# CaptainCuong/Efficient-GNN

Measured on NVIDIA B200. Metric: chebyshev_wavelet_nnz_k_f_per_s, higher is better.
Workload: dtype f32

## Files before the change

### efficient-gnn_b200/_cabi.py

```python
from __future__ import annotations

import ctypes as C
import os
import threading

_HERE = os.path.dirname(os.path.abspath(__file__))
LIB_PATH = os.environ.get("EGNN_LIB_PATH") or os.path.join(_HERE, "lib", "libegnn_b200.so")
ABI_VERSION = 9

_P, _I32, _I64, _F32, _SZ = C.c_void_p, C.c_int32, C.c_int64, C.c_float, C.c_size_t
SYMBOLS = {
    "egnn_abi_version": (C.c_int, []),
    "egnn_last_error": (C.c_char_p, []),
    "egnn_device_info": (C.c_int, [_P, _P, _P]),
    "egnn_dense_to_csr_count": (C.c_int, [_P, _I64, _I64, _P, _P, _P]),
    "egnn_dense_to_csr_fill": (C.c_int, [_P, _I64, _I64, _P, _P, _P, _P]),
    "egnn_graph_prep": (C.c_int, [_P, _P, _P, _I64, _P, _P, _P, _P, _P, _P, _P, _P, _P]),
    "egnn_degree_rows": (C.c_int, [_P, _P, _P, _I64, _I64, _I64, _P, _P, _P, _P, _P]),
    "egnn_graph_prep_finish": (C.c_int, [_P, _P, _P, _I64, _P, _P, _P, _P, _P]),
    "egnn_calibration_metrics_ws_bytes": (_SZ, [_I32, _I32]),
    "egnn_calibration_metrics": (C.c_int, [_P, _I32, _P, _P, _I64, _I32, _I32, _P, _P, _SZ, _P]),
    "egnn_temperature_head": (C.c_int, [_P, _P, _P, _P, _P, _P, _P, _P, _I64, _I32, _I32, _I32, _P]),
    "egnn_gcn_propagate": (C.c_int, [_P, _P, _P, _P, _P, _P, _P, _I64, _I32, _P, _P, _P, _I32, _P]),
    "egnn_gcn_target_logits": (C.c_int, [_P, _P, _P, _P, _P, _P, _I32, _I64, _I32, _I32, _P, _P, _P, _P, _P, _I32, _P]),
# ... 45 lines not shown
                                          _I32, _I32, _P, _P, _P, _I32, _P]),
    "egnn_cheb_adjoint_sharded": (C.c_int, [_P, _P, _P, _P, _P, _P, _P, _P, _P, _P, _P, _P, _P,
                                            _I64, _I64, _I64, _I64, _I32, _I32, _I32, _I32, _P, _F32, _F32, _I32,
                                            _P, _P, _P, _I32, _P]),
    "egnn_wide_adjoint_sharded": (C.c_int, [_P, _P, _P, _P, _P, _P, _P, _P, _I64, _I64, _I64, _I32, _I32, _I32, _I32,
                                            _P, _F32, _F32, _P, _P, _P, _I32, _P, _P]),
}


class SellPlanStruct(C.Structure):
    _fields_ = [("n", C.c_int32), ("n_blocks", C.c_int32), ("col_block", C.c_int32), ("lmax", C.c_int32),
                ("n_cols", C.c_int32), ("row0", C.c_int32), ("n_cta", C.c_int32), ("reserved", C.c_int32),
                ("n_slices", C.c_int64), ("n_vrows", C.c_int64), ("n_entries", C.c_int64), ("n_rowv", C.c_int64),
                ("slice_off", C.c_void_p), ("blk_slice_ptr", C.c_void_p), ("idx", C.c_void_p),
                ("rv_ptr", C.c_void_p), ("vslot", C.c_void_p), ("cta_info", C.c_void_p), ("vpart", C.c_void_p),
                ("sched", C.c_void_p), ("stamps", C.c_void_p)]


MAX_RANKS = 16
IPC_HANDLE_BYTES = 64


class PeerWindowStruct(C.Structure):
    _fields_ = [("rank", C.c_int32), ("world", C.c_int32), ("rows_per", C.c_int64), ("f", C.c_int32),
                ("reserved", C.c_int32), ("base", C.c_void_p * MAX_RANKS)]


class EgnnError(RuntimeError):
    """A non-zero status from libegnn_b200 (message from egnn_last_error)."""


# ... 72 lines not shown
```

### efficient-gnn_b200/csrc/egnn_cabi.cu

```cuda
#include <stdarg.h>
#include <stdlib.h>

#include "adjoint.cuh"
#include "cheb.cuh"
#include "common.cuh"
#include "head.cuh"
#include "metrics.cuh"
#include "peer.cuh"
#include "prep.cuh"
#include "sell.cuh"
#include "sell_step.cuh"
#include "structure_grad.cuh"
#include "surrogate.cuh"
#include "blocked.cuh"
#include "wide.cuh"

namespace egnn {

static thread_local char g_err[512] = {0};
char* last_error_buf() { return g_err; }
void set_error(const char* fmt, ...) {
    va_list ap;
    va_start(ap, fmt);
    vsnprintf(g_err, sizeof(g_err), fmt, ap);
// ... 220 lines not shown
static void fill_peer_push(PeerPush& pp, const egnn_peer_window* w, int which, bool has_data, bool wait_first) {
    pp.world = w->world; pp.rank = w->rank; pp.wait_first = wait_first; pp.has_data = has_data;
    char* own = (char*)w->base[w->rank];
    for (int r = 0; r < w->world; ++r) {
        pp.dst[r] = peer_operand(w, r, which);
        pp.flag[r] = (unsigned*)((char*)w->base[r] + kPeerFlagsOff) + w->rank;
    }
    pp.local_flags = (unsigned*)(own + kPeerFlagsOff);
    pp.epoch = (unsigned*)(own + kPeerEpochOff);
    pp.done_ctr = (unsigned*)(own + kPeerDoneOff);
    pp.error = (unsigned*)(own + kPeerErrorOff);
}

static void step_fill_plan(SellStepParams& sp, const egnn_sell_plan* pl) {
    sp.idx = pl->idx; sp.slice_off = pl->slice_off; sp.blk_slice_ptr = pl->blk_slice_ptr; sp.vslot = pl->vslot;
    sp.cta_info = pl->cta_info; sp.rv_ptr = pl->rv_ptr; sp.vpart = pl->vpart; sp.sched = pl->sched;
    sp.stamps = (unsigned long long*)pl->stamps;
    sp.trace = pl->reserved;
    sp.n_cta = pl->n_cta; sp.C = pl->n_blocks; sp.CB = pl->col_block; sp.n_cols = pl->n_cols;
    sp.n_rows = pl->n; sp.row0 = pl->row0;
}

static void step_fill_peer(SellStepParams& sp, const egnn_peer_window* w) {
    sp.world = w->world; sp.rank = w->rank; sp.rows_per = w->rows_per;
    char* own = (char*)w->base[w->rank];
    for (int r = 0; r < w->world; ++r) sp.flag_at[r] = (unsigned*)((char*)w->base[r] + kPeerFlagsOff) + w->rank;
    sp.local_flags = (unsigned*)(own + kPeerFlagsOff);
    sp.epoch = (unsigned*)(own + kPeerEpochOff);
    sp.error = (unsigned*)(own + kPeerErrorOff);
}

// ... 35 lines not shown
    return EGNN_OK;
}

static int device_sm_count() {
    int dev = 0, sms = kSmCountB200;
    if (cudaGetDevice(&dev) == cudaSuccess) cudaDeviceGetAttribute(&sms, cudaDevAttrMultiProcessorCount, dev);
    return sms;
}

}

using namespace egnn;

extern "C" {

int egnn_abi_version(void) { return 9; }

const char* egnn_last_error(void) { return last_error_buf(); }

int egnn_device_info(int32_t* sm_count, int32_t* cc_major, int32_t* cc_minor) {
    int dev = 0;
    int rc = check_cuda(cudaGetDevice(&dev), "cudaGetDevice");
    if (rc) return rc;
    cudaDeviceProp prop;
    rc = check_cuda(cudaGetDeviceProperties(&prop, dev), "cudaGetDeviceProperties");
    if (rc) return rc;
    if (sm_count) *sm_count = prop.multiProcessorCount;
    if (cc_major) *cc_major = prop.major;
    if (cc_minor) *cc_minor = prop.minor;
    if (prop.major != 10) {
        set_error("libegnn_b200 is built for sm_100a only; device is sm_%d%d", prop.major, prop.minor);
// ... 248 lines not shown
    float* tbuf[2] = {(float*)ws, (float*)(ws + slab)};
    float* ybuf[2] = {(float*)(ws + 2 * slab), (float*)(ws + 3 * slab)};

    if (t_all_or_null) {
        rc = check_cuda(cudaMemcpyAsync(t_all_or_null, x0, sizeof(float) * slab_elems, cudaMemcpyDeviceToDevice, st), "copy T0");
        if (rc) return rc;
    }
    if (cfg.prescaled && !sell_plan) {
        prescale_kernel<<<grid_for((int64_t)slab_elems, 256), 256, 0, st>>>(x0, dinv, ybuf[0], n, f, 0);
        EGNN_LAUNCH_CHECK("prescale_kernel launch");
    }

    if (sell_plan) {
        EGNN_REQUIRE(f == 1 && vals_or_null == nullptr, "the SELL plan serves F = 1 on a binary adjacency");
        EGNN_REQUIRE(sell_plan->n == n && sell_plan->n_cols == n && sell_plan->row0 == 0 && sell_plan->vpart && sell_plan->slice_off && sell_plan->blk_slice_ptr &&
                     sell_plan->rv_ptr && sell_plan->vslot && sell_plan->cta_info && sell_plan->sched, "SELL plan does not match the graph or is not filled");
        SellStepParams sp{};
        step_fill_plan(sp, sell_plan);
        sp.delta = p.delta;
        sp.w_base = w_base_or_null; sp.rowsum_base = rowsum_base_or_null; sp.patch_x0 = default_signal ? 1 : 0;
        sp.dinv = dinv; sp.iso = iso; sp.x0 = x0;
        sp.operand_first = y0_or_null;
        sp.operand[0] = ybuf[0]; sp.operand[1] = ybuf[1];
        sp.ydst[0][0] = ybuf[0]; sp.ydst[1][0] = ybuf[1]; sp.n_dst = 1;
        sp.tbuf[0] = tbuf[0]; sp.tbuf[1] = tbuf[1]; sp.t_all = t_all_or_null; sp.out = out;
        sp.normalize = normalize_l1; sp.a = op_scale; sp.b = op_shift;
        sp.world = 1; sp.rank = 0; sp.rows_per = n;
        if (order_events_host) {
            rc = check_cuda(cudaEventRecord((cudaEvent_t)order_events_host[0], st), "event record");
            if (rc) return rc;
        }
// ... 615 lines not shown
    rc = check_cuda(cub::DeviceScan::ExclusiveSum(w.cub_temp, tb, w.nvrow, w.rv_ptr, (int)(n + 1), st), "scan nvrow"); if (rc) return rc;
    sell_emit_kernel<<<(unsigned)ceil_div64(cn, 256), 256, 0, st>>>((int)n, C, lmax, w.seg_start, w.seg_cnt, w.nv, w.u_off,
                                                                   w.rv_ptr, w.key, w.uval, w.vsrc, w.vslot, w.vrow);
    EGNN_LAUNCH_CHECK("sell_emit_kernel launch");
    tb = w.cub_bytes;
    rc = check_cuda(cub::DeviceRadixSort::SortPairs(w.cub_temp, tb, w.key, w.key_sorted, w.uval, w.perm, (int)w.umax, 0, 32, st), "sort vrows");
    if (rc) return rc;
    sell_blocks_kernel<<<1, 32, 0, st>>>((int)n, C, w.u_off, w.q_ptr, w.vp_ptr, w.bsp, w.bstride, w.totals);
    EGNN_LAUNCH_CHECK("sell_blocks_kernel launch");
    sell_slice_kernel<<<(unsigned)ceil_div64(w.smax, 256), 256, 0, st>>>(C, lmax, w.key_sorted, w.q_ptr, w.bsp, w.bstride, w.totals, w.slice_sz);
    EGNN_LAUNCH_CHECK("sell_slice_kernel launch");
    tb = w.cub_bytes;
    rc = check_cuda(cub::DeviceScan::ExclusiveSum(w.cub_temp, tb, w.slice_sz, w.slice_off, (int)(w.smax + 1), st), "scan slices"); if (rc) return rc;
    sell_totals_kernel<<<1, 32, 0, st>>>(w.slice_off, w.rv_ptr, (int)n, w.totals);
    EGNN_LAUNCH_CHECK("sell_totals_kernel launch");
    int64_t tot[8];
    rc = check_cuda(cudaMemcpyAsync(tot, w.totals, 64, cudaMemcpyDeviceToHost, st), "copy totals"); if (rc) return rc;
    rc = check_cuda(cudaStreamSynchronize(st), "sync"); if (rc) return rc;
    plan->n = (int32_t)n;
    plan->n_cta = device_sm_count();
    plan->n_vrows = tot[kTotV];
    plan->n_slices = tot[kTotSlices];
    plan->n_entries = tot[kTotEntries];
    plan->n_rowv = tot[kTotRowV];
    return EGNN_OK;
}

int egnn_sell_fill(const int32_t* rowptr, const int32_t* colidx, int64_t n, int64_t nnz,
                   const egnn_sell_plan* plan, void* workspace, size_t workspace_bytes, egnn_stream_t stream) {
    int rc = sell_check_geometry(n, nnz, plan);
    if (rc) return rc;
    (void)rowptr;
    EGNN_REQUIRE(plan->slice_off && plan->blk_slice_ptr && plan->rv_ptr && plan->cta_info && plan->sched, "plan buffers not allocated");
    EGNN_REQUIRE(plan->n_cta >= 1 && plan->n_cta <= 4096, "n_cta out of range");
    EGNN_REQUIRE(plan->n_entries == 0 || plan->idx, "plan idx not allocated");
    EGNN_REQUIRE(plan->n_vrows == 0 || plan->vslot, "plan vslot not allocated");
    const int C = plan->n_blocks, CB = plan->col_block, lmax = plan->lmax;
    SellWs w = sell_ws_layout(workspace, n, nnz, C, lmax);
    if (!workspace || workspace_bytes < w.total_bytes) {
        set_error("sell workspace too small: need %zu bytes, got %zu", w.total_bytes, workspace_bytes);
        return EGNN_ERR_WORKSPACE;
    }
    cudaStream_t st = (cudaStream_t)stream;
    rc = check_cuda(cudaMemcpyAsync(plan->slice_off, w.slice_off, 4 * (plan->n_slices + 1), cudaMemcpyDeviceToDevice, st), "copy slice_off"); if (rc) return rc;
    rc = check_cuda(cudaMemcpyAsync(plan->blk_slice_ptr, w.bsp, 4 * (C + 1), cudaMemcpyDeviceToDevice, st), "copy blk_slice_ptr"); if (rc) return rc;
    rc = check_cuda(cudaMemcpyAsync(plan->rv_ptr, w.rv_ptr, 4 * (n + 1), cudaMemcpyDeviceToDevice, st), "copy rv_ptr"); if (rc) return rc;
    sell_cta_blocks_kernel<<<1, 32, 0, st>>>(w.slice_off, w.bsp, C, plan->n_cta, plan->cta_info, plan->sched);
    EGNN_LAUNCH_CHECK("sell_cta_blocks_kernel launch");
    sell_row_cost_kernel<<<(unsigned)ceil_div64(n + 1, 256), 256, 0, st>>>(w.rv_ptr, (int)n, w.nvrow);
    EGNN_LAUNCH_CHECK("sell_row_cost_kernel launch");
    size_t tb = w.cub_bytes;
    rc = check_cuda(cub::DeviceScan::ExclusiveSum(w.cub_temp, tb, w.nvrow, w.nv, (int)(n + 1), st), "scan row costs"); if (rc) return rc;
    sell_cta_rows_kernel<<<(unsigned)ceil_div64(plan->n_cta + 1, 128), 128, 0, st>>>(w.nv, (int)n, plan->n_cta,
                                                                                 plan->cta_info + 2 * plan->n_cta + kSellMaxBlocks);
    EGNN_LAUNCH_CHECK("sell_cta_rows_kernel launch");
    if (plan->n_slices > 0) {
        rc = check_cuda(cudaFuncSetAttribute(sell_fill_kernel, cudaFuncAttributeMaxDynamicSharedMemorySize, (int)kSellFillSmem),
                        "cudaFuncSetAttribute(sell_fill_kernel)");
        if (rc) return rc;
        sell_fill_kernel<<<(unsigned)ceil_div64(plan->n_slices, kSellFillWarps), kSellFillWarps * 32, kSellFillSmem, st>>>(
            colidx, C, CB, lmax, (int)plan->n_slices, w.key_sorted, w.perm, w.vsrc, w.vslot, w.vrow, w.q_ptr, w.vp_ptr,
            w.bsp, w.bstride, w.slice_off, plan->idx, plan->vslot, plan->row0);
        EGNN_LAUNCH_CHECK("sell_fill_kernel launch");
    }
    return EGNN_OK;
}

int egnn_sell_step_sharded(const egnn_sell_plan* plan, const float* dinv_full, const uint8_t* iso_full,
                           const float* x0_local, const float* y_first_full, float* y_slab0, float* y_slab1,
                           float* tbuf0, float* tbuf1, float* t_all_or_null, float* out_local,
                           int32_t order_begin, int32_t order_end, int32_t k_max, int32_t n_scales,
                           const float* coeffs_host, float op_scale, float op_shift, int32_t normalize_l1,
                           const int32_t* delta_row_host, const int32_t* delta_col_host,
                           const float* delta_val_host, int32_t n_delta,
                           const float* w_base_or_null, const float* rowsum_base_or_null, int32_t default_signal,
                           const egnn_peer_window* win, egnn_stream_t stream) {
    EGNN_REQUIRE(plan && dinv_full && iso_full && out_local && coeffs_host, "null pointer");
    EGNN_REQUIRE((w_base_or_null == nullptr) == (rowsum_base_or_null == nullptr), "w_base and rowsum_base come together");
    EGNN_REQUIRE(plan->vpart && plan->slice_off && plan->blk_slice_ptr && plan->rv_ptr && plan->vslot && plan->cta_info && plan->sched,
                 "SELL plan is not filled");
    EGNN_REQUIRE(order_begin >= 1 && order_begin <= order_end && order_end <= k_max && k_max <= EGNN_MAX_ORDER, "bad order range");
    EGNN_REQUIRE(n_scales >= 1 && n_scales <= EGNN_MAX_SCALES, "n_scales out of range");
    EGNN_REQUIRE(plan->n == 0 || x0_local, "T_0 rows missing");
    EGNN_REQUIRE(t_all_or_null || k_max == 1 || (tbuf0 && tbuf1), "T buffers missing");
    const bool fused = win && win->world > 1;
    if (win) {
        int rc = peer_check(win);
        if (rc) return rc;
        EGNN_REQUIRE(win->f == 1 && (int64_t)win->world * win->rows_per >= plan->n_cols &&
                     (int64_t)plan->row0 + plan->n <= (int64_t)win->world * win->rows_per, "window does not fit the plan");
    } else {
        EGNN_REQUIRE(plan->n == plan->n_cols || (order_begin == order_end && y_first_full),
                     "a row shard without an exchange window runs one order per call on a gathered operand");
        EGNN_REQUIRE(order_end == k_max || (y_slab0 && y_slab1), "operand slabs missing");
// ... 516 lines not shown
```

### efficient-gnn_b200/csrc/sell.cuh

```cuda
#pragma once

#include <cub/device/device_radix_sort.cuh>
#include <cub/device/device_scan.cuh>

#include "cheb.cuh"
#include "common.cuh"
#include "peer.cuh"

namespace egnn {

constexpr int kSellThreads = 1024;
constexpr int kSellThreadsPerCta = kSellThreads;
constexpr int kSellCtrStride = 32;
constexpr int kSellSchedWords = 64 * kSellCtrStride + 64;
constexpr int kSellSliceRows = 32;
constexpr int kSellGroup = 8;
constexpr int kSellMaxBlocks = 64;

enum SellTotals { kTotU = 0, kTotV = 1, kTotSlices = 2, kTotEntries = 3, kTotRowV = 4 };

__global__ void __launch_bounds__(256)
sell_count_kernel(const int32_t* __restrict__ rowptr, const int32_t* __restrict__ colidx, int n, int C,
                  int CB, int lmax, int32_t* __restrict__ seg_start, int32_t* __restrict__ seg_cnt,
                  int32_t* __restrict__ nv, int32_t* __restrict__ nvrow) {
    const int i = blockIdx.x * blockDim.x + threadIdx.x;
    if (i >= n) return;
    const int e = rowptr[i + 1];
    int prev = rowptr[i];
    int total = 0;
    for (int c = 0; c < C; ++c) {
        int pos = e;
        if (c + 1 < C) {
            const int bound = (c + 1) * CB;
            int lo = prev, hi = e;
// ... 119 lines not shown
    int g = 0, max_cnt = 0;
    for (int c = 0; c < C; ++c) max_cnt = max(max_cnt, cnt[c]);
    for (int r = 0; r < max_cnt; ++r)
        for (int c = 0; c < C; ++c)
            if (r < cnt[c]) { cta_info[g] = c; cta_info[n_cta + g] = r; ++g; }
    for (; g < n_cta; ++g) { cta_info[g] = -1; cta_info[n_cta + g] = 0; }
    for (int i = 0; i < kSellSchedWords; ++i) sched[i] = 0u;
    for (int c = 0; c < kSellMaxBlocks; ++c) {
        const int start = c < C ? cnt[c] * (kSellThreadsPerCta / 32) : 0;
        cta_info[2 * n_cta + c] = start;
        sched[c * kSellCtrStride] = (unsigned)start;
    }
}

constexpr int kSellEpiWarpRow = 24;
__global__ void sell_row_cost_kernel(const int32_t* __restrict__ rv_ptr, int n, int32_t* __restrict__ cost) {
    const int i = blockIdx.x * blockDim.x + threadIdx.x;
    if (i > n) return;
    if (i == n) { cost[i] = 0; return; }
    const int parts = rv_ptr[i + 1] - rv_ptr[i];
    cost[i] = parts > kSellEpiWarpRow ? 28 + parts / 8 : 4;
}

__global__ void sell_cta_rows_kernel(const int32_t* __restrict__ cost_prefix, int n, int n_cta, int32_t* __restrict__ cta_rows) {
    const int g = blockIdx.x * blockDim.x + threadIdx.x;
    if (g > n_cta) return;
    if (g == 0) { cta_rows[0] = 0; return; }
    if (g == n_cta) { cta_rows[g] = n; return; }
    const int64_t target = (int64_t)cost_prefix[n] * g / n_cta;
    int lo = 0, hi = n;
    while (lo < hi) {
        const int mid = (lo + hi) >> 1;
        if (cost_prefix[mid] < target) lo = mid + 1; else hi = mid;
    }
    cta_rows[g] = lo;
}

__global__ void sell_totals_kernel(const int32_t* __restrict__ slice_off, const int32_t* __restrict__ rv_ptr,
                                   int n, int64_t* __restrict__ totals) {
    if (threadIdx.x != 0 || blockIdx.x != 0) return;
    totals[kTotEntries] = slice_off[totals[kTotSlices]];
    totals[kTotRowV] = rv_ptr[n];
}

constexpr int kSellFillWarps = 8;
constexpr int kSellLmaxCap = 256;
constexpr int kSellMaskWords = kSellLmaxCap / 32;
constexpr size_t kSellFillSmem = (size_t)kSellFillWarps * 32 * kSellMaskWords * sizeof(uint32_t);

__global__ void __launch_bounds__(kSellFillWarps * 32)
// ... 113 lines not shown
```

### efficient-gnn_b200/csrc/sell_step.cuh

```cuda
#pragma once

#include "common.cuh"
#include "peer.cuh"
#include "prep.cuh"
#include "sell.cuh"

namespace egnn {

constexpr int kStepMaxOrders = 16;
constexpr int kSchedBarrier = kSellMaxBlocks * kSellCtrStride;
constexpr int kEpiWarpRow = kSellEpiWarpRow;
constexpr int kStageChunkFloats = 8192;

struct SellStepParams {
    const uint16_t* idx;
    const int32_t* slice_off;
    const int32_t* blk_slice_ptr;
    const int32_t* vslot;
    const int32_t* cta_info;
    const int32_t* rv_ptr;
    float* vpart;
    unsigned* sched;
    unsigned long long* stamps;
    int32_t trace;
    int32_t n_cta, C, CB, n_cols, n_rows, row0;
    const float* dinv;
    const uint8_t* iso;
    const float* x0;
    const float* operand_first;
    const float* operand[2];
    float* ydst[2][EGNN_MAX_RANKS];
    int32_t n_dst;
    float* tbuf[2];
    float* t_all;
// ... 97 lines not shown
        if (node[j] == gi) return j;
    return -1;
}

__device__ __forceinline__ const float* step_t_ptr(const SellStepParams& p, int j) {
    if (j == 0) return p.x0;
    return p.t_all ? p.t_all + (size_t)j * p.n_rows : p.tbuf[(j - 1) & 1];
}

struct StepRowPre {
    int t, e;
    float di, theta, xprev, t2, out0;
};

template <bool PATCH>
__device__ __forceinline__ StepRowPre step_row_prefetch(const SellStepParams& p, const StepOrderView& v, int i) {
    StepRowPre r;
    const int gi = p.row0 + i;
    r.t = __ldg(p.rv_ptr + i);
    r.e = __ldg(p.rv_ptr + i + 1);
    r.di = __ldg(p.dinv + gi);
    r.theta = fmaf(p.a, 1.f - (float)__ldg(p.iso + gi), p.b);
    r.xprev = v.tprev[i];
    r.t2 = v.first ? 0.f : v.tprev2[i];
    r.out0 = v.first ? 0.f : p.out[(size_t)i * p.S];
    if (PATCH && v.touched_here) {
        const int j = step_patch_find(v.pt_node, v.n_touch, gi);
        if (j >= 0) {
            r.di = v.pt_dinv[j];
            r.theta = fmaf(p.a, 1.f - (float)v.pt_iso[j], p.b);
            if (v.k == 1) r.xprev = v.pt_x0[j];
            if (v.k == 2) r.t2 = v.pt_x0[j];
        }
    }
    return r;
}

__device__ __forceinline__ void step_epilogue_finish(const SellStepParams& p, const StepOrderView& v, int i,
                                                     const StepRowPre& r, double accd) {
    const int gi = p.row0 + i;
    if (v.flips_here)
        for (int d = 0; d < p.delta.n; ++d)
            if (p.delta.row[d] == gi) accd += (double)v.flip_term[d];
    const float acc = (float)accd;
    const float lap = fmaf(r.theta, r.xprev, -p.a * r.di * acc);
    const float tk = v.first ? lap : fmaf(2.f, lap, -r.t2);
    if (v.tk) v.tk[i] = tk;
    if (v.push) {
        const float yv = r.di * tk;
        for (int d = 0; d < p.n_dst; ++d) p.ydst[v.k & 1][d][gi] = yv;
    }
    for (int s = 0; s < p.S; ++s) {
        float o = v.first ? fmaf(p.coef[s][v.j + 1], tk, p.coef[s][v.j] * r.xprev)
                          : fmaf(p.coef[s][v.j + 1], tk, s == 0 ? r.out0 : p.out[(size_t)i * p.S + s]);
        if (v.last && p.normalize) o = o / (fabsf(o) + 1e-8f);
        p.out[(size_t)i * p.S + s] = o;
    }
}

__device__ __forceinline__ double step_row_sum(const float* vpart, int t, int e) {
    double a = 0.0;
    for (; t < e; t += 8) {
        float x[8];
#pragma unroll
        for (int u = 0; u < 8; ++u) x[u] = t + u < e ? __ldcg(vpart + t + u) : 0.f;
#pragma unroll
        for (int u = 0; u < 8; ++u) a += (double)x[u];
    }
    return a;
}

template <bool PEER, bool PATCH>
__global__ void __launch_bounds__(kSellThreads, 1)
sell_step_kernel(const __grid_constant__ SellStepParams p) {
    extern __shared__ __align__(128) float ysm[];
    __shared__ __align__(8) unsigned long long stage_bar;
    __shared__ int hub_cnt;
    __shared__ float flip_term[EGNN_MAX_DELTA];
    __shared__ int pt_node[PATCH ? 2 * EGNN_MAX_DELTA : 1];
    __shared__ float pt_dinv[PATCH ? 2 * EGNN_MAX_DELTA : 1], pt_x0[PATCH ? 2 * EGNN_MAX_DELTA : 1], pt_y0[PATCH ? 2 * EGNN_MAX_DELTA : 1];
    __shared__ unsigned char pt_iso[PATCH ? 2 * EGNN_MAX_DELTA : 1];
    const int tid = threadIdx.x;
    const int lane = tid & 31;
    const int wid = tid >> 5;
    constexpr int kWarps = kSellThreads / 32;
    const int g = blockIdx.x;
    const unsigned n_cta = gridDim.x;

    const int c = __ldg(p.cta_info + g);
    const int rank_in_block = __ldg(p.cta_info + p.n_cta + g);
    int bs0 = 0, bs1 = 0, ctas_in_block = 1;
    if (c >= 0) {
        bs0 = __ldg(p.blk_slice_ptr + c);
        bs1 = __ldg(p.blk_slice_ptr + c + 1);
        ctas_in_block = __ldg(p.cta_info + 2 * p.n_cta + c) / (kSellThreads / 32);
    }
    const bool has_slices = c >= 0 && bs1 > bs0;
    const int col0 = c >= 0 ? c * p.CB : 0;
    const int cnt = c >= 0 ? min(p.CB, p.n_cols - col0) : 0;
#ifdef EGNN_EQUAL_EPILOGUE_ROWS
    const int r0 = (int)((int64_t)p.n_rows * g / p.n_cta);
    const int r1 = (int)((int64_t)p.n_rows * (g + 1) / p.n_cta);
#else
    const int r0 = __ldg(p.cta_info + 2 * p.n_cta + kSellMaxBlocks + g);
    const int r1 = __ldg(p.cta_info + 2 * p.n_cta + kSellMaxBlocks + g + 1);
#endif

    unsigned long long* bar_ctr = reinterpret_cast<unsigned long long*>(p.sched + kSchedBarrier);
    unsigned long long bar_base = 0;
    unsigned epoch_base = 0;
    if (tid == 0) {
        const unsigned long long seen = ld_relaxed_gpu_u64(bar_ctr);
        bar_base = seen - seen % n_cta;
        mbar_init(&stage_bar, 1);
        if (p.stamps && g == 0) p.stamps[0] = global_timer_ns();
    }
    if (PEER) epoch_base = *p.epoch;
    unsigned bar_done = 0;
    unsigned signals = 0;
    unsigned stage_parity = 0;
    int stamp_i = 1;
    bool pending = false, pending_signal = false;
    const bool late_done = PEER && p.delta.n > 0;
    const int n_touch = PATCH ? 2 * p.delta.n : 0;
    bool touched_here = false;
    if (PATCH) {
        if (tid < n_touch) {
            const int u = tid < p.delta.n ? p.delta.row[tid] : p.delta.col[tid - p.delta.n];
            float dw = 0.f, dr = 0.f;
            for (int j = 0; j < p.delta.n; ++j) {
                if (p.delta.col[j] == u && p.delta.row[j] != u) dw += p.delta.val[j];
                if (p.delta.row[j] == u) dr += p.delta.val[j];
            }
            float dv;
            uint8_t is;
            normaliser_from_w(__ldg(p.w_base + u) + dw, dv, is);
// ... 13 lines not shown

    auto wait_windows_free = [&]() {
        if (PEER && wid == 0) peer_wait_ranks(p.local_flags, 0, p.world - 1, p.rank, epoch_base + signals, p.error, false, lane);
    };
    auto signal_peers = [&]() {
        signals += 1u;
        if (PEER && g == 0 && tid == 0) {
            const unsigned e = epoch_base + signals;
            *p.epoch = e;
            __threadfence_system();
            for (int q = 0; q < p.world; ++q)
                if (q != p.rank) st_relaxed_sys_u32(p.flag_at[q], e);
        }
    };
    auto stamp = [&]() {
        if (p.stamps && g == 0 && tid == 0) p.stamps[stamp_i] = global_timer_ns();
        ++stamp_i;
    };
    int trace_i = 0;
    auto trace = [&]() {
        if (p.stamps && p.trace && tid == 0 && trace_i < 64) p.stamps[64 + (size_t)g * 64 + trace_i] = global_timer_ns();
        ++trace_i;
    };
    auto bar_arrive = [&](bool sys_scope) {
        __syncthreads();
        if (tid == 0) grid_arrive(bar_ctr, sys_scope);
    };
    auto bar_wait = [&]() {
        if (tid == 0) grid_wait(bar_ctr, bar_base + (unsigned long long)(bar_done + 1u) * n_cta);
        bar_done += 1u;
        __syncthreads();
    };
    auto finish_pending = [&]() {
        if (pending) {
            bar_wait();
            if (pending_signal) signal_peers();
            stamp();
// ... 100 lines not shown
                    for (int u = 0; u < kSellUnroll; ++u) q[u] = ld_stream_u32x4(q0 + (size_t)(gq + u) * kSellSliceRows);
#pragma unroll
                    for (int u = 0; u < kSellUnroll; ++u) {
                        if (u & 1) acc1 += sell_gather8(ysm, q[u]);
                        else acc0 += sell_gather8(ysm, q[u]);
                    }
                }
                for (; gq < groups; ++gq) acc0 += sell_gather8(ysm, ld_stream_u32x4(q0 + (size_t)gq * kSellSliceRows));
                if (slot >= 0) p.vpart[slot] = acc0 + acc1;
                s = s_next; off = off_next; end = end_next; slot = slot_next;
            }
        }
        bar_arrive(false);
        trace();

        int* hub_list = reinterpret_cast<int*>(ysm);
        const int hub_cap = p.CB;
        if (tid == 0) hub_cnt = 0;
        const int i_a = r0 + tid, i_b = r0 + tid + kSellThreads;
        StepRowPre pre_a{}, pre_b{};
        if (i_a < r1) pre_a = step_row_prefetch<PATCH>(p, v, i_a);
        if (i_b < r1) pre_b = step_row_prefetch<PATCH>(p, v, i_b);
        if (PEER && (v.push || flips_here)) {
            wait_windows_free();
            if (flips_here) __syncthreads();
        }
        if (flips_here && tid < p.delta.n) {
            const int lr = p.delta.row[tid] - p.row0, dc = p.delta.col[tid];
            const float yc = (PATCH && held && k == 1) ? pt_y0[p.delta.n + tid] : __ldcg(v.operand + dc);
            flip_term[tid] = (lr >= r0 && lr < r1 && dc != p.delta.row[tid]) ? p.delta.val[tid] * yc : 0.f;
        }
        bar_wait();
        stamp();
        if (PEER && v.last && !late_done) signal_peers();
        if (g == 0 && tid < p.C) p.sched[tid * kSellCtrStride] = (unsigned)__ldg(p.cta_info + 2 * p.n_cta + tid);
        for (int i = i_a; i < r1; i += kSellThreads) {
            const StepRowPre r = i == i_a ? pre_a : (i == i_b ? pre_b : step_row_prefetch<PATCH>(p, v, i));
            if (r.e - r.t > kEpiWarpRow) {
                const int h = atomicAdd(&hub_cnt, 1);
                if (h < hub_cap) { hub_list[h] = i; continue; }
            }
            step_epilogue_finish(p, v, i, r, step_row_sum(p.vpart, r.t, r.e));
        }
        __syncthreads();
        const int n_hub = min(hub_cnt, hub_cap);
        for (int h = wid; h < n_hub; h += kWarps) {
            const int i = hub_list[h];
            const StepRowPre r = step_row_prefetch<PATCH>(p, v, i);
            double a = 0.0;
            for (int t = r.t + lane; t < r.e; t += 32) a += (double)__ldcg(p.vpart + t);
#pragma unroll
            for (int o = 16; o > 0; o >>= 1) a += __shfl_xor_sync(0xffffffffu, a, o);
            if (lane == 0) step_epilogue_finish(p, v, i, r, a);
        }
        if (k < p.order_end || (PEER && (v.push || (v.last && late_done)))) {
            bar_arrive(PEER && v.push);
            pending = true; pending_signal = v.push || (v.last && late_done);
        }
        trace();
    }
    finish_pending();
    if (p.stamps && g == 0 && tid == 0) p.stamps[stamp_i] = global_timer_ns();
}

}
```

### efficient-gnn_b200/graph.py

```python
from __future__ import annotations

import ctypes as C
from typing import Optional, Sequence

import numpy as np
import torch

from . import _cabi

__all__ = ["CsrGraph", "as_graph", "deltas_from_dense", "enable_phase_stamps", "read_phase_stamps"]


def _stream():
    return _cabi.current_stream()


class CsrGraph:

    def __init__(self, rowptr: torch.Tensor, colidx: torch.Tensor, vals: Optional[torch.Tensor], n: int,
                 _prepare: bool = True):
        _cabi.require_device()
        if rowptr.dtype != torch.int32 or colidx.dtype != torch.int32:
            raise TypeError("rowptr/colidx must be int32")
        if not (rowptr.is_cuda and colidx.is_cuda):
# ... 287 lines not shown
    with torch.cuda.device(dev):
        plan = _cabi.SellPlanStruct()
        plan.n, plan.n_blocks, plan.col_block, plan.lmax = n_rows, nb, cb, lmax
        plan.n_cols, plan.row0 = n_cols, row0
        ws_bytes = int(lib.egnn_sell_ws_bytes(n_rows, nnz, nb, lmax))
        ws = torch.empty(ws_bytes, dtype=torch.uint8, device=dev)
        _cabi.check(lib.egnn_sell_prepare(_cabi.ptr(rowptr), _cabi.ptr(colidx), n_rows, nnz,
                                          C.byref(plan), _cabi.ptr(ws), ws_bytes, _stream()), "egnn_sell_prepare")
        bufs = {
            "slice_off": torch.empty(plan.n_slices + 1, dtype=torch.int32, device=dev),
            "blk_slice_ptr": torch.empty(plan.n_blocks + 1, dtype=torch.int32, device=dev),
            "idx": torch.empty(max(1, plan.n_entries), dtype=torch.int16, device=dev),
            "rv_ptr": torch.empty(n_rows + 1, dtype=torch.int32, device=dev),
            "vslot": torch.empty(max(1, plan.n_vrows), dtype=torch.int32, device=dev),
            "cta_info": torch.empty(3 * plan.n_cta + 65, dtype=torch.int32, device=dev),
            "vpart": torch.empty(max(1, plan.n_rowv), dtype=torch.float32, device=dev),
            "sched": torch.zeros(64 * 32 + 64, dtype=torch.int32, device=dev),
        }
        for name, t in bufs.items():
            setattr(plan, name, t.data_ptr())
        _cabi.check(lib.egnn_sell_fill(_cabi.ptr(rowptr), _cabi.ptr(colidx), n_rows, nnz,
                                       C.byref(plan), _cabi.ptr(ws), ws_bytes, _stream()), "egnn_sell_fill")
    plan._keepalive = bufs
    return plan


def enable_phase_stamps(plan, on: bool = True, trace: bool = False):
    if on:
        if "stamps" not in plan._keepalive:
            plan._keepalive["stamps"] = torch.zeros(64 + 64 * plan.n_cta, dtype=torch.int64,
# ... 62 lines not shown
```

### include/egnn_b200.h

```cpp
#ifndef EGNN_B200_H
#define EGNN_B200_H

#include <stddef.h>
#include <stdint.h>

#ifdef __cplusplus
extern "C" {
#endif

typedef void* egnn_stream_t;

enum egnn_status {
    EGNN_OK = 0,
    EGNN_ERR_INVALID_ARG = -1,
    EGNN_ERR_CUDA = -2,
    EGNN_ERR_UNSUPPORTED_ARCH = -3,
    EGNN_ERR_WORKSPACE = -4
};

#define EGNN_MAX_SCALES 8
#define EGNN_MAX_ORDER 64
#define EGNN_MAX_DELTA 64
#define EGNN_MAX_RANKS 16
#define EGNN_IPC_HANDLE_BYTES 64
// ... 43 lines not shown

typedef struct egnn_sell_plan {
    int32_t n, n_blocks, col_block, lmax;
    int32_t n_cols, row0;
    int32_t n_cta, reserved;
    int64_t n_slices, n_vrows, n_entries, n_rowv;
    int32_t* slice_off;
    int32_t* blk_slice_ptr;
    uint16_t* idx;
    int32_t* rv_ptr;
    int32_t* vslot;
    int32_t* cta_info;
    float* vpart;
    uint32_t* sched;
    uint64_t* stamps;
} egnn_sell_plan;

int egnn_sell_geometry(int64_t n_cols, int64_t nnz, int32_t* n_blocks, int32_t* col_block, int32_t* lmax);
size_t egnn_sell_ws_bytes(int64_t n, int64_t nnz, int32_t n_blocks, int32_t lmax);
int egnn_sell_prepare(const int32_t* rowptr, const int32_t* colidx, int64_t n, int64_t nnz,
                      egnn_sell_plan* plan, void* workspace, size_t workspace_bytes,
                      egnn_stream_t stream);
int egnn_sell_fill(const int32_t* rowptr, const int32_t* colidx, int64_t n, int64_t nnz,
                   const egnn_sell_plan* plan, void* workspace, size_t workspace_bytes,
                   egnn_stream_t stream);

size_t egnn_cheb_workspace_bytes(int64_t n, int32_t f);
int egnn_cheb_wavelet(const int32_t* rowptr, const int32_t* colidx,
                      const float* vals_or_null, const float* dinv,
                      const uint8_t* iso, const float* x0, int64_t n, int64_t nnz,
// ... 195 lines not shown
```

Measured before the change: 2074 billion.

## Precompute per-CTA hub row lists and overlap hub epilogue loads with row prefetch

Builds the list of high-degree (hub) rows for each CTA during plan fill, so the SELL step kernel no longer discovers hubs at runtime with a shared atomic counter and a __syncthreads. Each warp prefetches its first hub row's metadata lane-parallel and issues the first partial-sum loads for normal and hub rows early, so more memory requests are in flight at once. The stamp and trace counters move to shared memory. The cost is extra plan-build kernels, an added plan buffer and an ABI bump, plus more register use in the step kernel.

```diff
diff --git a/efficient-gnn_b200/_cabi.py b/efficient-gnn_b200/_cabi.py
--- a/efficient-gnn_b200/_cabi.py
+++ b/efficient-gnn_b200/_cabi.py
@@ -6,7 +6,7 @@
 
 _HERE = os.path.dirname(os.path.abspath(__file__))
 LIB_PATH = os.environ.get("EGNN_LIB_PATH") or os.path.join(_HERE, "lib", "libegnn_b200.so")
-ABI_VERSION = 9
+ABI_VERSION = 10
 
 _P, _I32, _I64, _F32, _SZ = C.c_void_p, C.c_int32, C.c_int64, C.c_float, C.c_size_t
 SYMBOLS = {
@@ -83,7 +83,7 @@
                 ("n_slices", C.c_int64), ("n_vrows", C.c_int64), ("n_entries", C.c_int64), ("n_rowv", C.c_int64),
                 ("slice_off", C.c_void_p), ("blk_slice_ptr", C.c_void_p), ("idx", C.c_void_p),
                 ("rv_ptr", C.c_void_p), ("vslot", C.c_void_p), ("cta_info", C.c_void_p), ("vpart", C.c_void_p),
-                ("sched", C.c_void_p), ("stamps", C.c_void_p)]
+                ("sched", C.c_void_p), ("stamps", C.c_void_p), ("n_hub", C.c_int64), ("hub", C.c_void_p)]
 
 
 MAX_RANKS = 16
diff --git a/efficient-gnn_b200/csrc/egnn_cabi.cu b/efficient-gnn_b200/csrc/egnn_cabi.cu
--- a/efficient-gnn_b200/csrc/egnn_cabi.cu
+++ b/efficient-gnn_b200/csrc/egnn_cabi.cu
@@ -258,7 +258,7 @@
 
 static void step_fill_plan(SellStepParams& sp, const egnn_sell_plan* pl) {
     sp.idx = pl->idx; sp.slice_off = pl->slice_off; sp.blk_slice_ptr = pl->blk_slice_ptr; sp.vslot = pl->vslot;
-    sp.cta_info = pl->cta_info; sp.rv_ptr = pl->rv_ptr; sp.vpart = pl->vpart; sp.sched = pl->sched;
+    sp.cta_info = pl->cta_info; sp.hub = pl->hub; sp.rv_ptr = pl->rv_ptr; sp.vpart = pl->vpart; sp.sched = pl->sched;
     sp.stamps = (unsigned long long*)pl->stamps;
     sp.trace = pl->reserved;
     sp.n_cta = pl->n_cta; sp.C = pl->n_blocks; sp.CB = pl->col_block; sp.n_cols = pl->n_cols;
@@ -324,7 +324,7 @@
 
 extern "C" {
 
-int egnn_abi_version(void) { return 9; }
+int egnn_abi_version(void) { return 10; }
 
 const char* egnn_last_error(void) { return last_error_buf(); }
 
@@ -603,7 +603,7 @@
     if (sell_plan) {
         EGNN_REQUIRE(f == 1 && vals_or_null == nullptr, "the SELL plan serves F = 1 on a binary adjacency");
         EGNN_REQUIRE(sell_plan->n == n && sell_plan->n_cols == n && sell_plan->row0 == 0 && sell_plan->vpart && sell_plan->slice_off && sell_plan->blk_slice_ptr &&
-                     sell_plan->rv_ptr && sell_plan->vslot && sell_plan->cta_info && sell_plan->sched, "SELL plan does not match the graph or is not filled");
+                     sell_plan->rv_ptr && sell_plan->vslot && sell_plan->cta_info && sell_plan->hub && sell_plan->sched, "SELL plan does not match the graph or is not filled");
         SellStepParams sp{};
         step_fill_plan(sp, sell_plan);
         sp.delta = p.delta;
@@ -1249,6 +1249,8 @@
     rc = check_cuda(cub::DeviceScan::ExclusiveSum(w.cub_temp, tb, w.slice_sz, w.slice_off, (int)(w.smax + 1), st), "scan slices"); if (rc) return rc;
     sell_totals_kernel<<<1, 32, 0, st>>>(w.slice_off, w.rv_ptr, (int)n, w.totals);
     EGNN_LAUNCH_CHECK("sell_totals_kernel launch");
+    sell_hub_count_kernel<<<(unsigned)ceil_div64(n, 256), 256, 0, st>>>(w.rv_ptr, (int)n, w.totals);
+    EGNN_LAUNCH_CHECK("sell_hub_count_kernel launch");
     int64_t tot[8];
     rc = check_cuda(cudaMemcpyAsync(tot, w.totals, 64, cudaMemcpyDeviceToHost, st), "copy totals"); if (rc) return rc;
     rc = check_cuda(cudaStreamSynchronize(st), "sync"); if (rc) return rc;
@@ -1258,6 +1260,7 @@
     plan->n_slices = tot[kTotSlices];
     plan->n_entries = tot[kTotEntries];
     plan->n_rowv = tot[kTotRowV];
+    plan->n_hub = tot[kTotHub];
     return EGNN_OK;
 }
 
@@ -1266,7 +1269,9 @@
     int rc = sell_check_geometry(n, nnz, plan);
     if (rc) return rc;
     (void)rowptr;
-    EGNN_REQUIRE(plan->slice_off && plan->blk_slice_ptr && plan->rv_ptr && plan->cta_info && plan->sched, "plan buffers not allocated");
+    EGNN_REQUIRE(plan->slice_off && plan->blk_slice_ptr && plan->rv_ptr && plan->cta_info && plan->sched && plan->hub,
+                 "plan buffers not allocated");
+    EGNN_REQUIRE(plan->n_hub >= 0 && plan->n_hub <= n, "n_hub out of range");
     EGNN_REQUIRE(plan->n_cta >= 1 && plan->n_cta <= 4096, "n_cta out of range");
     EGNN_REQUIRE(plan->n_entries == 0 || plan->idx, "plan idx not allocated");
     EGNN_REQUIRE(plan->n_vrows == 0 || plan->vslot, "plan vslot not allocated");
@@ -1282,13 +1287,20 @@
     rc = check_cuda(cudaMemcpyAsync(plan->rv_ptr, w.rv_ptr, 4 * (n + 1), cudaMemcpyDeviceToDevice, st), "copy rv_ptr"); if (rc) return rc;
     sell_cta_blocks_kernel<<<1, 32, 0, st>>>(w.slice_off, w.bsp, C, plan->n_cta, plan->cta_info, plan->sched);
     EGNN_LAUNCH_CHECK("sell_cta_blocks_kernel launch");
-    sell_row_cost_kernel<<<(unsigned)ceil_div64(n + 1, 256), 256, 0, st>>>(w.rv_ptr, (int)n, w.nvrow);
+    int32_t* hub_flag = w.u_off;
+    int32_t* hub_prefix = reinterpret_cast<int32_t*>(w.key);
+    int32_t* cta_rows = plan->cta_info + 2 * plan->n_cta + kSellMaxBlocks;
+    sell_row_cost_kernel<<<(unsigned)ceil_div64(n + 1, 256), 256, 0, st>>>(w.rv_ptr, (int)n, w.nvrow, hub_flag);
     EGNN_LAUNCH_CHECK("sell_row_cost_kernel launch");
     size_t tb = w.cub_bytes;
     rc = check_cuda(cub::DeviceScan::ExclusiveSum(w.cub_temp, tb, w.nvrow, w.nv, (int)(n + 1), st), "scan row costs"); if (rc) return rc;
-    sell_cta_rows_kernel<<<(unsigned)ceil_div64(plan->n_cta + 1, 128), 128, 0, st>>>(w.nv, (int)n, plan->n_cta,
-                                                                                 plan->cta_info + 2 * plan->n_cta + kSellMaxBlocks);
+    sell_cta_rows_kernel<<<(unsigned)ceil_div64(plan->n_cta + 1, 128), 128, 0, st>>>(w.nv, (int)n, plan->n_cta, cta_rows);
     EGNN_LAUNCH_CHECK("sell_cta_rows_kernel launch");
+    tb = w.cub_bytes;
+    rc = check_cuda(cub::DeviceScan::ExclusiveSum(w.cub_temp, tb, hub_flag, hub_prefix, (int)(n + 1), st), "scan hub flags"); if (rc) return rc;
+    sell_cta_hubs_kernel<<<(unsigned)ceil_div64(n > plan->n_cta ? n : plan->n_cta + 1, 256), 256, 0, st>>>(
+        hub_flag, hub_prefix, cta_rows, (int)n, plan->n_cta, plan->hub);
+    EGNN_LAUNCH_CHECK("sell_cta_hubs_kernel launch");
     if (plan->n_slices > 0) {
         rc = check_cuda(cudaFuncSetAttribute(sell_fill_kernel, cudaFuncAttributeMaxDynamicSharedMemorySize, (int)kSellFillSmem),
                         "cudaFuncSetAttribute(sell_fill_kernel)");
@@ -1312,7 +1324,7 @@
                            const egnn_peer_window* win, egnn_stream_t stream) {
     EGNN_REQUIRE(plan && dinv_full && iso_full && out_local && coeffs_host, "null pointer");
     EGNN_REQUIRE((w_base_or_null == nullptr) == (rowsum_base_or_null == nullptr), "w_base and rowsum_base come together");
-    EGNN_REQUIRE(plan->vpart && plan->slice_off && plan->blk_slice_ptr && plan->rv_ptr && plan->vslot && plan->cta_info && plan->sched,
+    EGNN_REQUIRE(plan->vpart && plan->slice_off && plan->blk_slice_ptr && plan->rv_ptr && plan->vslot && plan->cta_info && plan->hub && plan->sched,
                  "SELL plan is not filled");
     EGNN_REQUIRE(order_begin >= 1 && order_begin <= order_end && order_end <= k_max && k_max <= EGNN_MAX_ORDER, "bad order range");
     EGNN_REQUIRE(n_scales >= 1 && n_scales <= EGNN_MAX_SCALES, "n_scales out of range");
diff --git a/efficient-gnn_b200/csrc/sell.cuh b/efficient-gnn_b200/csrc/sell.cuh
--- a/efficient-gnn_b200/csrc/sell.cuh
+++ b/efficient-gnn_b200/csrc/sell.cuh
@@ -17,7 +17,7 @@
 constexpr int kSellGroup = 8;
 constexpr int kSellMaxBlocks = 64;
 
-enum SellTotals { kTotU = 0, kTotV = 1, kTotSlices = 2, kTotEntries = 3, kTotRowV = 4 };
+enum SellTotals { kTotU = 0, kTotV = 1, kTotSlices = 2, kTotEntries = 3, kTotRowV = 4, kTotHub = 5 };
 
 __global__ void __launch_bounds__(256)
 sell_count_kernel(const int32_t* __restrict__ rowptr, const int32_t* __restrict__ colidx, int n, int C,
@@ -167,12 +167,25 @@
 }
 
 constexpr int kSellEpiWarpRow = 24;
-__global__ void sell_row_cost_kernel(const int32_t* __restrict__ rv_ptr, int n, int32_t* __restrict__ cost) {
+__device__ __forceinline__ bool sell_is_hub_row(const int32_t* rv_ptr, int i) {
+    return rv_ptr[i + 1] - rv_ptr[i] > kSellEpiWarpRow;
+}
+
+__global__ void sell_row_cost_kernel(const int32_t* __restrict__ rv_ptr, int n, int32_t* __restrict__ cost,
+                                     int32_t* __restrict__ hub) {
     const int i = blockIdx.x * blockDim.x + threadIdx.x;
     if (i > n) return;
-    if (i == n) { cost[i] = 0; return; }
+    if (i == n) { cost[i] = 0; hub[i] = 0; return; }
     const int parts = rv_ptr[i + 1] - rv_ptr[i];
     cost[i] = parts > kSellEpiWarpRow ? 28 + parts / 8 : 4;
+    hub[i] = parts > kSellEpiWarpRow ? 1 : 0;
+}
+
+__global__ void sell_hub_count_kernel(const int32_t* __restrict__ rv_ptr, int n, int64_t* __restrict__ totals) {
+    const int i = blockIdx.x * blockDim.x + threadIdx.x;
+    const bool hub = i < n && sell_is_hub_row(rv_ptr, i);
+    const unsigned m = __ballot_sync(0xffffffffu, hub);
+    if ((threadIdx.x & 31) == 0 && m) atomicAdd(reinterpret_cast<unsigned long long*>(totals + kTotHub), (unsigned long long)__popc(m));
 }
 
 __global__ void sell_cta_rows_kernel(const int32_t* __restrict__ cost_prefix, int n, int n_cta, int32_t* __restrict__ cta_rows) {
@@ -187,6 +200,13 @@
         if (cost_prefix[mid] < target) lo = mid + 1; else hi = mid;
     }
     cta_rows[g] = lo;
+}
+
+__global__ void sell_cta_hubs_kernel(const int32_t* __restrict__ hub_flag, const int32_t* __restrict__ hub_prefix,
+                                     const int32_t* __restrict__ cta_rows, int n, int n_cta, int32_t* __restrict__ hub) {
+    const int i = blockIdx.x * blockDim.x + threadIdx.x;
+    if (i <= n_cta) hub[i] = hub_prefix[cta_rows[i]];
+    if (i < n && hub_flag[i]) hub[n_cta + 1 + hub_prefix[i]] = i;
 }
 
 __global__ void sell_totals_kernel(const int32_t* __restrict__ slice_off, const int32_t* __restrict__ rv_ptr,
diff --git a/efficient-gnn_b200/csrc/sell_step.cuh b/efficient-gnn_b200/csrc/sell_step.cuh
--- a/efficient-gnn_b200/csrc/sell_step.cuh
+++ b/efficient-gnn_b200/csrc/sell_step.cuh
@@ -11,6 +11,7 @@
 constexpr int kSchedBarrier = kSellMaxBlocks * kSellCtrStride;
 constexpr int kEpiWarpRow = kSellEpiWarpRow;
 constexpr int kStageChunkFloats = 8192;
+constexpr int kEpiFirstParts = 5;
 
 struct SellStepParams {
     const uint16_t* idx;
@@ -18,6 +19,7 @@
     const int32_t* blk_slice_ptr;
     const int32_t* vslot;
     const int32_t* cta_info;
+    const int32_t* hub;
     const int32_t* rv_ptr;
     float* vpart;
     unsigned* sched;
@@ -145,6 +147,19 @@
 };
 
 template <bool PATCH>
+__device__ __forceinline__ void step_row_patch(const SellStepParams& p, const StepOrderView& v, int gi, StepRowPre& r) {
+    if (PATCH && v.touched_here) {
+        const int j = step_patch_find(v.pt_node, v.n_touch, gi);
+        if (j >= 0) {
+            r.di = v.pt_dinv[j];
+            r.theta = fmaf(p.a, 1.f - (float)v.pt_iso[j], p.b);
+            if (v.k == 1) r.xprev = v.pt_x0[j];
+            if (v.k == 2) r.t2 = v.pt_x0[j];
+        }
+    }
+}
+
+template <bool PATCH>
 __device__ __forceinline__ StepRowPre step_row_prefetch(const SellStepParams& p, const StepOrderView& v, int i) {
     StepRowPre r;
     const int gi = p.row0 + i;
@@ -155,15 +170,33 @@
     r.xprev = v.tprev[i];
     r.t2 = v.first ? 0.f : v.tprev2[i];
     r.out0 = v.first ? 0.f : p.out[(size_t)i * p.S];
-    if (PATCH && v.touched_here) {
-        const int j = step_patch_find(v.pt_node, v.n_touch, gi);
-        if (j >= 0) {
-            r.di = v.pt_dinv[j];
-            r.theta = fmaf(p.a, 1.f - (float)v.pt_iso[j], p.b);
-            if (v.k == 1) r.xprev = v.pt_x0[j];
-            if (v.k == 2) r.t2 = v.pt_x0[j];
-        }
-    }
+    step_row_patch<PATCH>(p, v, gi, r);
+    return r;
+}
+
+__device__ __forceinline__ uint32_t step_hub_prefetch(const SellStepParams& p, const StepOrderView& v, int i, int lane) {
+    const int gi = p.row0 + i;
+    uint32_t w = 0u;
+    if (lane == 0) w = (uint32_t)__ldg(p.rv_ptr + i);
+    else if (lane == 1) w = (uint32_t)__ldg(p.rv_ptr + i + 1);
+    else if (lane == 2) w = __float_as_uint(__ldg(p.dinv + gi));
+    else if (lane == 3) w = __ldg(p.iso + gi);
+    else if (lane == 4) w = __float_as_uint(v.tprev[i]);
+    else if (lane == 5 && !v.first) w = __float_as_uint(v.tprev2[i]);
+    else if (lane == 6 && !v.first) w = __float_as_uint(p.out[(size_t)i * p.S]);
+    return w;
+}
+template <bool PATCH>
+__device__ __forceinline__ StepRowPre step_hub_gather(const SellStepParams& p, const StepOrderView& v, int i, uint32_t w) {
+    StepRowPre r;
+    r.t = (int)__shfl_sync(0xffffffffu, w, 0);
+    r.e = (int)__shfl_sync(0xffffffffu, w, 1);
+    r.di = __uint_as_float(__shfl_sync(0xffffffffu, w, 2));
+    r.theta = fmaf(p.a, 1.f - (float)__shfl_sync(0xffffffffu, w, 3), p.b);
+    r.xprev = __uint_as_float(__shfl_sync(0xffffffffu, w, 4));
+    r.t2 = __uint_as_float(__shfl_sync(0xffffffffu, w, 5));
+    r.out0 = __uint_as_float(__shfl_sync(0xffffffffu, w, 6));
+    step_row_patch<PATCH>(p, v, p.row0 + i, r);
     return r;
 }
 
@@ -189,16 +222,41 @@
     }
 }
 
-__device__ __forceinline__ double step_row_sum(const float* vpart, int t, int e) {
+template <int N>
+__device__ __forceinline__ void step_row_load(const float* vpart, int t, int e, float (&x)[N]) {
+#pragma unroll
+    for (int u = 0; u < N; ++u) x[u] = t + u < e ? __ldcg(vpart + t + u) : 0.f;
+}
+template <int N>
+__device__ __forceinline__ double step_row_sum_rest(const float* vpart, int t, int e, const float (&x0)[N]) {
     double a = 0.0;
-    for (; t < e; t += 8) {
+#pragma unroll
+    for (int u = 0; u < N; ++u) a += (double)x0[u];
+    for (t += N; t < e; t += 8) {
         float x[8];
-#pragma unroll
-        for (int u = 0; u < 8; ++u) x[u] = t + u < e ? __ldcg(vpart + t + u) : 0.f;
+        step_row_load(vpart, t, e, x);
 #pragma unroll
         for (int u = 0; u < 8; ++u) a += (double)x[u];
     }
     return a;
+}
+__device__ __forceinline__ double step_row_sum(const float* vpart, int t, int e) {
+    float x[8];
+    step_row_load(vpart, t, e, x);
+    return step_row_sum_rest(vpart, t, e, x);
+}
+
+__device__ __forceinline__ void step_hub_finish(const SellStepParams& p, const StepOrderView& v, int i,
+                                                const StepRowPre& r, float x0, int lane) {
+    double a = 0.0;
+    a += (double)x0;
+    for (int t = r.t + lane + 32; t < r.e; t += 32) a += (double)__ldcg(p.vpart + t);
+#pragma unroll
+    for (int o = 16; o > 0; o >>= 1) a += __shfl_xor_sync(0xffffffffu, a, o);
+    if (lane == 0) step_epilogue_finish(p, v, i, r, a);
+}
+__device__ __forceinline__ float step_hub_first(const float* vpart, int t, int e, int lane) {
+    return t + lane < e ? __ldcg(vpart + t + lane) : 0.f;
 }
 
 template <bool PEER, bool PATCH>
@@ -206,7 +264,7 @@
 sell_step_kernel(const __grid_constant__ SellStepParams p) {
     extern __shared__ __align__(128) float ysm[];
     __shared__ __align__(8) unsigned long long stage_bar;
-    __shared__ int hub_cnt;
+    __shared__ int hub_first[kSellThreads / 32], hub_span[2];
     __shared__ float flip_term[EGNN_MAX_DELTA];
     __shared__ int pt_node[PATCH ? 2 * EGNN_MAX_DELTA : 1];
     __shared__ float pt_dinv[PATCH ? 2 * EGNN_MAX_DELTA : 1], pt_x0[PATCH ? 2 * EGNN_MAX_DELTA : 1], pt_y0[PATCH ? 2 * EGNN_MAX_DELTA : 1];
@@ -229,20 +287,23 @@
     const bool has_slices = c >= 0 && bs1 > bs0;
     const int col0 = c >= 0 ? c * p.CB : 0;
     const int cnt = c >= 0 ? min(p.CB, p.n_cols - col0) : 0;
-#ifdef EGNN_EQUAL_EPILOGUE_ROWS
-    const int r0 = (int)((int64_t)p.n_rows * g / p.n_cta);
-    const int r1 = (int)((int64_t)p.n_rows * (g + 1) / p.n_cta);
-#else
     const int r0 = __ldg(p.cta_info + 2 * p.n_cta + kSellMaxBlocks + g);
     const int r1 = __ldg(p.cta_info + 2 * p.n_cta + kSellMaxBlocks + g + 1);
-#endif
+    if (tid < kWarps) {
+        const int hb = __ldg(p.hub + g), he = __ldg(p.hub + g + 1);
+        hub_first[tid] = hb + tid < he ? __ldg(p.hub + p.n_cta + 1 + hb + tid) : -1;
+        if (tid == 0) { hub_span[0] = hb; hub_span[1] = he; }
+    }
 
     unsigned long long* bar_ctr = reinterpret_cast<unsigned long long*>(p.sched + kSchedBarrier);
-    unsigned long long bar_base = 0;
+    __shared__ unsigned long long bar_base;
+    __shared__ int stamp_i, trace_i;
     unsigned epoch_base = 0;
     if (tid == 0) {
         const unsigned long long seen = ld_relaxed_gpu_u64(bar_ctr);
         bar_base = seen - seen % n_cta;
+        stamp_i = 1;
+        trace_i = 0;
         mbar_init(&stage_bar, 1);
         if (p.stamps && g == 0) p.stamps[0] = global_timer_ns();
     }
@@ -250,7 +311,6 @@
     unsigned bar_done = 0;
     unsigned signals = 0;
     unsigned stage_parity = 0;
-    int stamp_i = 1;
     bool pending = false, pending_signal = false;
     const bool late_done = PEER && p.delta.n > 0;
     const int n_touch = PATCH ? 2 * p.delta.n : 0;
@@ -294,13 +354,16 @@
         }
     };
     auto stamp = [&]() {
-        if (p.stamps && g == 0 && tid == 0) p.stamps[stamp_i] = global_timer_ns();
-        ++stamp_i;
-    };
-    int trace_i = 0;
+        if (tid == 0) {
+            if (p.stamps && g == 0) p.stamps[stamp_i] = global_timer_ns();
+            ++stamp_i;
+        }
+    };
     auto trace = [&]() {
-        if (p.stamps && p.trace && tid == 0 && trace_i < 64) p.stamps[64 + (size_t)g * 64 + trace_i] = global_timer_ns();
-        ++trace_i;
+        if (tid == 0) {
+            if (p.stamps && p.trace && trace_i < 64) p.stamps[64 + (size_t)g * 64 + trace_i] = global_timer_ns();
+            ++trace_i;
+        }
     };
     auto bar_arrive = [&](bool sys_scope) {
         __syncthreads();
@@ -431,13 +494,12 @@
         bar_arrive(false);
         trace();
 
-        int* hub_list = reinterpret_cast<int*>(ysm);
-        const int hub_cap = p.CB;
-        if (tid == 0) hub_cnt = 0;
         const int i_a = r0 + tid, i_b = r0 + tid + kSellThreads;
+        const int i_h = hub_first[wid];
         StepRowPre pre_a{}, pre_b{};
         if (i_a < r1) pre_a = step_row_prefetch<PATCH>(p, v, i_a);
         if (i_b < r1) pre_b = step_row_prefetch<PATCH>(p, v, i_b);
+        const uint32_t wh = i_h >= 0 ? step_hub_prefetch(p, v, i_h, lane) : 0u;
         if (PEER && (v.push || flips_here)) {
             wait_windows_free();
             if (flips_here) __syncthreads();
@@ -451,24 +513,26 @@
         stamp();
         if (PEER && v.last && !late_done) signal_peers();
         if (g == 0 && tid < p.C) p.sched[tid * kSellCtrStride] = (unsigned)__ldg(p.cta_info + 2 * p.n_cta + tid);
-        for (int i = i_a; i < r1; i += kSellThreads) {
-            const StepRowPre r = i == i_a ? pre_a : (i == i_b ? pre_b : step_row_prefetch<PATCH>(p, v, i));
-            if (r.e - r.t > kEpiWarpRow) {
-                const int h = atomicAdd(&hub_cnt, 1);
-                if (h < hub_cap) { hub_list[h] = i; continue; }
-            }
-            step_epilogue_finish(p, v, i, r, step_row_sum(p.vpart, r.t, r.e));
-        }
-        __syncthreads();
-        const int n_hub = min(hub_cnt, hub_cap);
-        for (int h = wid; h < n_hub; h += kWarps) {
-            const int i = hub_list[h];
+        const bool own_a = i_a < r1 && pre_a.e - pre_a.t <= kEpiWarpRow;
+        const bool own_b = i_b < r1 && pre_b.e - pre_b.t <= kEpiWarpRow;
+        float xa[kEpiFirstParts], xb[kEpiFirstParts];
+        step_row_load(p.vpart, pre_a.t, own_a ? pre_a.e : pre_a.t, xa);
+        step_row_load(p.vpart, pre_b.t, own_b ? pre_b.e : pre_b.t, xb);
+        const float xh = i_h >= 0 ? step_hub_first(p.vpart, (int)__shfl_sync(0xffffffffu, wh, 0),
+                                                   (int)__shfl_sync(0xffffffffu, wh, 1), lane) : 0.f;
+        if (own_a) step_epilogue_finish(p, v, i_a, pre_a, step_row_sum_rest(p.vpart, pre_a.t, pre_a.e, xa));
+        if (own_b) step_epilogue_finish(p, v, i_b, pre_b, step_row_sum_rest(p.vpart, pre_b.t, pre_b.e, xb));
+        for (int i = i_b + kSellThreads; i < r1; i += kSellThreads) {
             const StepRowPre r = step_row_prefetch<PATCH>(p, v, i);
-            double a = 0.0;
-            for (int t = r.t + lane; t < r.e; t += 32) a += (double)__ldcg(p.vpart + t);
-#pragma unroll
-            for (int o = 16; o > 0; o >>= 1) a += __shfl_xor_sync(0xffffffffu, a, o);
-            if (lane == 0) step_epilogue_finish(p, v, i, r, a);
+            if (r.e - r.t <= kEpiWarpRow) step_epilogue_finish(p, v, i, r, step_row_sum(p.vpart, r.t, r.e));
+        }
+        if (i_h >= 0) {
+            step_hub_finish(p, v, i_h, step_hub_gather<PATCH>(p, v, i_h, wh), xh, lane);
+            for (int h = hub_span[0] + wid + kWarps; h < hub_span[1]; h += kWarps) {
+                const int i = __ldg(p.hub + p.n_cta + 1 + h);
+                const StepRowPre r = step_row_prefetch<PATCH>(p, v, i);
+                step_hub_finish(p, v, i, r, step_hub_first(p.vpart, r.t, r.e, lane), lane);
+            }
         }
         if (k < p.order_end || (PEER && (v.push || (v.last && late_done)))) {
             bar_arrive(PEER && v.push);
diff --git a/efficient-gnn_b200/graph.py b/efficient-gnn_b200/graph.py
--- a/efficient-gnn_b200/graph.py
+++ b/efficient-gnn_b200/graph.py
@@ -325,6 +325,7 @@
             "rv_ptr": torch.empty(n_rows + 1, dtype=torch.int32, device=dev),
             "vslot": torch.empty(max(1, plan.n_vrows), dtype=torch.int32, device=dev),
             "cta_info": torch.empty(3 * plan.n_cta + 65, dtype=torch.int32, device=dev),
+            "hub": torch.empty(plan.n_cta + 1 + plan.n_hub, dtype=torch.int32, device=dev),
             "vpart": torch.empty(max(1, plan.n_rowv), dtype=torch.float32, device=dev),
             "sched": torch.zeros(64 * 32 + 64, dtype=torch.int32, device=dev),
         }
diff --git a/include/egnn_b200.h b/include/egnn_b200.h
--- a/include/egnn_b200.h
+++ b/include/egnn_b200.h
@@ -81,6 +81,8 @@
     float* vpart;
     uint32_t* sched;
     uint64_t* stamps;
+    int64_t n_hub;
+    int32_t* hub;
 } egnn_sell_plan;
 
 int egnn_sell_geometry(int64_t n_cols, int64_t nnz, int32_t* n_blocks, int32_t* col_block, int32_t* lmax);
```

Measured after the change: 2194 billion, median of 6. 1.06x the previous value.
